# jsourati/nn-active-learning

Hardware: AMD Instinct MI355X
Metric: patches/sec Fisher-scored (32^3, 2-class) (higher is better)
Workload: dtype f32 (fp32 operands split into 16-bit pieces on the 16-bit MFMA, fp32 accumulate: fp16 pairs - 22-23 bits kept per operand, three products - in the conv under the head (forward + backward), in dec1's forward launch and in the other backward launches; bf16 triples - all 24 bits, exact, six products -

## Files before the change

include/alq.h:

```cpp
#ifndef ALQ_H
#define ALQ_H

#include <stddef.h>
#include <stdint.h>

#ifdef __cplusplus
extern "C" {
#endif

typedef struct alq_ctx alq_ctx;
typedef struct alq_model alq_model;

enum { ALQ_OK = 0, ALQ_EINVAL = -1, ALQ_EHIP = -2, ALQ_ENOMEM = -3, ALQ_EUNSUPPORTED = -4 };

enum { ALQ_CONV = 0, ALQ_CONVT = 1, ALQ_POOL = 2, ALQ_FC = 3 };

typedef struct {
    int32_t type;
    int32_t cout;
    int32_t k[3];
    int32_t s[3];
    int32_t relu;
    int32_t skip_src;
} alq_layer_t;
// ... 238 lines not shown

int alq_model_debug_copy(alq_model *m, int layer_idx, int what, int N, float *d_out,
                         int64_t *elems_out);

int alq_debug_set_stamp_buffer(void *d_buf);
int alq_debug_set(int key, int value);
enum {
    ALQ_INFO_SUBNORMALS_OK = 0,
    ALQ_INFO_C3D_FWD = 1,
    ALQ_INFO_C3D_BWD = 2,
    ALQ_INFO_C3D_ONE_ACC = 3,
    ALQ_INFO_FLIP_OVERFLOW = 5,
    ALQ_INFO_F16_DERIVED = 6,
    ALQ_INFO_T3D_FWD = 7,
    ALQ_INFO_T3D_BWD = 8,
    ALQ_INFO_E3D_BWD = 9,
    ALQ_INFO_D3D_FWD = 10,
    ALQ_INFO_D3D_BWD = 11,
    ALQ_INFO_F3D_FWD = 12,
    ALQ_INFO_C3D_BWD_FORM = 13,
    ALQ_INFO_HOST_PACK_ELEMS = 14,
    ALQ_INFO_LSUM = 15,
    ALQ_INFO_DCP_FORM = 16,
    ALQ_INFO_E3D_BWD_FORM = 17
};
int alq_model_engine_info(alq_model *m, int what);

int alq_synth_patches(alq_ctx *ctx, uint64_t seed, int64_t first_id, int64_t n,
                      int64_t elems_per_patch, float *d_out);

enum { ALQ_SRC_F32 = 0, ALQ_SRC_F64 = 1, ALQ_SRC_I16 = 2, ALQ_SRC_U8 = 3 };
int alq_vol_pack(alq_ctx *ctx, const void *const *d_src, int m, int src_type, const int32_t *dims, float *d_out);
int alq_mask_pack(alq_ctx *ctx, const uint8_t *d_src, const int32_t *dims, uint8_t *d_out);
int alq_slice_batch_check(const int32_t *h_dims, int nvol, const int32_t *h_desc, int b, const int32_t *crop, int C);
int alq_slice_batch(alq_ctx *ctx, const float *const *h_vols, const uint8_t *const *h_masks, const int32_t *h_dims, int nvol, int m,
                    const int32_t *h_desc, int b, const int32_t *crop, int C, float *d_X, int32_t *d_lab, int64_t *d_counts);
int64_t alq_slice_batch_trip_rows(void);
int alq_slice_batch_launch_samples(void);

#ifdef __cplusplus
}
#endif
#endif
```

nn-active-learning_amd/csrc/alq_internal.h:

```cpp
#pragma once
#include <hip/hip_runtime.h>

#include <cstdint>
#include <cstdio>
#include <memory>
#include <string>
#include <vector>

#include "alq.h"
#include "engine_switches.h"
#include "model_plan.h"

namespace alq {

#define ALQ_HIP(expr)                                                                     \
    do {                                                                                  \
        hipError_t e_ = (expr);                                                           \
        if (e_ != hipSuccess) {                                                           \
            ::alq::set_error("%s:%d: %s -> %s", __FILE__, __LINE__, #expr,               \
                             hipGetErrorString(e_));                                      \
            return ALQ_EHIP;                                                              \
        }                                                                                 \
    } while (0)

// ... 307 lines not shown
                  int relu, int accumulate, int N, int prof_cls, const Igemm2Fuse *fuse);

struct C3dPlan {
    bool ok = false;
    int D = 0;
    int w_exp = 0;
    int oneacc = 1;
    double flops_per_patch = 0;
    std::vector<unsigned short> h_W;
    void *d_W = nullptr;
    std::vector<unsigned short> h_W7;
    void *d_W7 = nullptr;
};
void c3d_bwd7_pack(C3dPlan *plan, const std::vector<float> &Bmat);
int c3d_subnormals_ok(alq_ctx *ctx);
int c3d_fwd_build(const View &in, const View &out, const int k[3], const int lo[3], const int s[3], C3dPlan *plan);
void c3d_fwd_pack(C3dPlan *plan, const std::vector<float> &Bmat );
int c3d_fwd_launch(alq_ctx *ctx, const C3dPlan &plan, const View &in, const float *bias, int N, const unsigned *amaxA, const unsigned *amaxB,
                   const float *fc_W, float *fc_part, float *asum_part, unsigned char *fc_bits, float flip_tau);
int c3d_bwd_build(const View &fwd_in, const View &fwd_out, const int k[3], const int lo[3], const int s[3], C3dPlan *plan);
void c3d_bwd_pack(C3dPlan *plan, const std::vector<float> &Bmat_fwd );
void c3d_presplit_vec(const float *v, long long F, int e, std::vector<unsigned short> *out);
int c3d_bwd_launch(alq_ctx *ctx, const C3dPlan &plan, int N, const unsigned char *bits, const void *vec16, int e_in, const unsigned char *maskA,
                   float *dB, float *sumA, float *sumB, int rows_per_wave = 8);

struct T3dPlan {
    bool ok = false;
    int kind = 0;
    int w_exp = 0;
    double flops_per_patch = 0;
    std::vector<unsigned short> h_W;
    void *d_W = nullptr;
};
int t3d_build(const View &in, const View &out, const int k[3], const int lo[3], const int s[3], T3dPlan *fwd, T3dPlan *bwd);
void t3d_fwd_pack(T3dPlan *plan, const float *W );
void t3d_bwd_pack(T3dPlan *plan, const float *W);
void t3d8_fwd_pack(T3dPlan *plan, const float *W );
void t3d8_bwd_pack(T3dPlan *plan, const float *W );
int t3d8_bwd_launch(alq_ctx *ctx, const T3dPlan &plan, const View &dout, const View &din, int N, float in_bound, const unsigned char *mask_bits, float *dsum);
int t3d_fwd_launch(alq_ctx *ctx, const T3dPlan &plan, const View &in, const View &out, const float *bias, int N, float *osum, unsigned *out_amax);
int t3d_bwd_launch(alq_ctx *ctx, const T3dPlan &plan, const View &dout, const View &din, int N, float in_bound, const unsigned char *mask_bits,
                   float *dsum);

struct E3dPlan {
    bool ok = false;
    int w_exp = 0;
    double flops_per_patch = 0;
// ... 275 lines not shown
```

nn-active-learning_amd/csrc/c3d.hip:

```cpp
#include "f16_pair.h"
#include "sweep_common.h"

#include <algorithm>
#include <cmath>
#include <cstdlib>
#include <cstring>
#include <vector>

namespace alq {

namespace {
#ifndef C3_SCHED_MASK
#define C3_SCHED_MASK 0
#endif
#ifndef C3_PF
#define C3_PF 8
#endif
#ifndef C3_WD
#define C3_WD 4
#endif
static_assert(C3_PF == 8 || C3_PF == 16, "the ring of staging registers must divide the 16 units of a plane");
static_assert(C3_WD >= 1 && C3_WD <= 8, "weight-difference slices are fetched 1..8 rows ahead");
#ifndef C3_ABL
#define C3_ABL 0
#endif
#ifndef C3_PIPE
#define C3_PIPE 2
#endif
#ifndef C3_FILL_MASK
#define C3_FILL_MASK SW_FILL_MASK
#endif
#ifndef C3_PIN_SUMS
#define C3_PIN_SUMS 1
#endif
#ifndef C3_PEEL
#define C3_PEEL 1
#endif
#ifndef C3_EPI2
#define C3_EPI2 1
#endif
#ifndef C3_BPIPE
#define C3_BPIPE 2
#endif
#ifndef C3_B7PIPE
#define C3_B7PIPE 4
#endif
#ifndef C3_B7PINW
#define C3_B7PINW 0
#endif
#ifndef C3_B7ABL
#define C3_B7ABL 0
#endif

constexpr int C3_TEN = 34 * 16;
constexpr int C3_PIECE = 2 * C3_TEN;
constexpr int C3_ROW = 2 * C3_PIECE;
constexpr int C3_PLANE = 34 * C3_ROW;
constexpr int C3_LDS = 2 * C3_PLANE;
static_assert(C3_LDS <= 160 * 1024, "two plane images must fit the CU's LDS");
}

struct C3FwdArgs {
    const float *inA, *inB;
    const void *W;
    const float *bias;
    const unsigned *amaxA, *amaxB;
    const float *fc_W;
    float *fc_part;
// ... 682 lines not shown
            step(IC<1>{}, pi, 3 * zz + 1, n); ++n;
            step(IC<2>{}, pi, 3 * zz + 2, n); ++n;
        }
        step(IC<0>{}, pi, 30, n); ++n;
        step(IC<1>{}, pi, 31, n); ++n;
        light(IC<0>{}, pi, D - 2);
#else
        for (int zz = 0; zz < 11; ++zz) {
            step(IC<0>{}, pi, 3 * zz, n); ++n;
            step(IC<1>{}, pi, 3 * zz + 1, n); ++n;
            if (zz < 10) { step(IC<2>{}, pi, 3 * zz + 2, n); ++n; }
            else light(IC<0>{}, pi, D - 2);
        }
#endif
    }
    if (np > 0) light(IC<1>{}, np - 1, D - 1);
}

namespace {
constexpr int P7_ROW = 34 * 16;
constexpr int P7_PIECE = 34 * P7_ROW;
constexpr int P7_PLANE = 2 * P7_PIECE + 128;
constexpr int P7_LDS = 4 * P7_PLANE;
static_assert((P7_ROW / 16) % 16 == 2 && (P7_PLANE / 16) % 16 == 0 && P7_LDS <= 160 * 1024, "bank-conflict-free pitches (see above)");
}

__global__ __launch_bounds__(256) __attribute__((amdgpu_waves_per_eu(1, 1))) void c3d_bwd7_kernel(const C3BwdArgs a) {
    extern __shared__ __attribute__((aligned(16))) char lds[];
    constexpr int RW = 8, NU = 4;
    const int tid = threadIdx.x;
    const int lane = tid & 63;
    const int wave = __builtin_amdgcn_readfirstlane(tid >> 6);
    const int lj = lane & 15, lq = lane >> 4;
    const int D = a.D;
    const unsigned plane_v = 32u * 32u;
    const unsigned patch_v = (unsigned)D * plane_v;

    for (int i = tid * 16; i < P7_LDS; i += 256 * 16) *reinterpret_cast<i32x4 *>(lds + i) = i32x4{0, 0, 0, 0};

    f16x8 Wa[3][2], Wb[3][2], Ws[2];
    {
        const i32x4 *Wg = reinterpret_cast<const i32x4 *>(a.W);
#pragma unroll
        for (int dz = 0; dz < 3; ++dz)
#pragma unroll
            for (int pc = 0; pc < 2; ++pc) {
                Wa[dz][pc] = __builtin_bit_cast(f16x8, Wg[((0 + dz) * 2 + pc) * 64 + lane]);
                Wb[dz][pc] = __builtin_bit_cast(f16x8, Wg[((3 + dz) * 2 + pc) * 64 + lane]);
            }
        Ws[0] = __builtin_bit_cast(f16x8, Wg[(6 * 2 + 0) * 64 + lane]);
        Ws[1] = __builtin_bit_cast(f16x8, Wg[(6 * 2 + 1) * 64 + lane]);
#if C3_B7PINW
#pragma unroll
        for (int dz = 0; dz < 3; ++dz)
#pragma unroll
            for (int pc = 0; pc < 2; ++pc) {
                i32x4 x = __builtin_bit_cast(i32x4, Wa[dz][pc]), y = __builtin_bit_cast(i32x4, Wb[dz][pc]);
                asm volatile("" : "+a"(x), "+a"(y));
                Wa[dz][pc] = __builtin_bit_cast(f16x8, x); Wb[dz][pc] = __builtin_bit_cast(f16x8, y);
            }
#endif
    }
    const int offA = wave * RW * P7_ROW + (lq < 3 ? (lj + lq) * 16 : P7_ROW + lj * 16);
    const int offB = (wave * RW + 1) * P7_ROW + (lq < 2 ? (lj + 1 + lq) * 16 : P7_ROW + (lj + lq - 2) * 16);
    const int offS = (wave * RW + 2) * P7_ROW + (lj + 2) * 16;
    const int ringS = lq < 2 ? lq + 2 : 0;
    const int st_lane = (wave * RW + 1 + (lane >> 5)) * P7_ROW + ((lane & 31) + 1) * 16;
    const float inv = __builtin_ldexpf(1.f, -(a.e_in + a.e_w));

    const int G = gridDim.x, b0 = blockIdx.x;
    const int np = b0 < a.N ? (a.N - b0 + G - 1) / G : 0;

    f32x4 acc[3][RW][2];
#pragma unroll
// ... 89 lines not shown
        const unsigned vox = E.pv + E.row_v + (unsigned)i * 32u + (unsigned)hx * 16u;
        __builtin_amdgcn_raw_buffer_store_b128(__builtin_bit_cast(i32x4, val), dB_rsrc, (int)E.off_dB, (int)(vox * 32u), 2 );
        if constexpr (!(C3_B7ABL & 8)) ALQ_STORE_HOLD("v"(val));
        const float t = (val.x + val.y) + (val.z + val.w);
        const unsigned tu = __builtin_bit_cast(unsigned, t);
        const auto sw = hx == 0 ? __builtin_amdgcn_permlane16_swap(tu, 0u, false, false) : __builtin_amdgcn_permlane16_swap(0u, tu, false, false);
        const unsigned s0 = sw[0], s1 = sw[1];
        const float t2 = __builtin_bit_cast(float, s0) + __builtin_bit_cast(float, s1);
        if constexpr (hx == 0) {
            t_keep = t2;
        } else {
            const float ts = t_keep + t2;
            const unsigned rowv = E.pv + E.row_v + (unsigned)i * 32u;
            __builtin_amdgcn_raw_buffer_store_b32(__builtin_bit_cast(int, ts), sA_rsrc, (int)(lq < 2 ? E.off_sum : SW_OOB), (int)(rowv * 4u), 0);
            __builtin_amdgcn_raw_buffer_store_b32(__builtin_bit_cast(int, ts), sB_rsrc, (int)(lq >= 2 ? E.off_sum : SW_OOB), (int)(rowv * 4u), 0);
        }
    };
    auto epi_row = [&](auto S, auto I, const Epi &E) __attribute__((always_inline)) {
        epi_half(S, I, IC<0>{}, E);
        epi_half(S, I, IC<1>{}, E);
    };
    auto s_weights = [&](int kill, f16x8 &sh, f16x8 &sl) __attribute__((always_inline)) {
        const int km = lq == kill ? 0 : -1;
        i32x4 h = __builtin_bit_cast(i32x4, Ws[0]), l = __builtin_bit_cast(i32x4, Ws[1]);
        h.x &= km; h.y &= km; h.z &= km; h.w &= km;
        l.x &= km; l.y &= km; l.z &= km; l.w &= km;
        sh = __builtin_bit_cast(f16x8, h); sl = __builtin_bit_cast(f16x8, l);
    };
    auto mac3 = [&](f32x4 c, const f16x8 &wh, const f16x8 &wl, const f16x8 &bh, const f16x8 &bl) __attribute__((always_inline)) {
        c = __builtin_amdgcn_mfma_f32_16x16x32_f16(wl, bh, c, 0, 0, 0);
        c = __builtin_amdgcn_mfma_f32_16x16x32_f16(wh, bl, c, 0, 0, 0);
        c = __builtin_amdgcn_mfma_f32_16x16x32_f16(wh, bh, c, 0, 0, 0);
        return c;
    };

    auto step = [&](auto RR, int pi, int z, long long n) __attribute__((always_inline)) {
        constexpr int R = decltype(RR)::value;
        constexpr int S_lo = (R + 2) % 3, S_mid = R, S_hi = (R + 1) % 3;
        asm volatile("s_waitcnt lgkmcnt(0)\n\ts_barrier" ::: "memory");
        const int cur = (int)(n & 3) * P7_PLANE;
        const int baseA = offA + cur, baseB = offB + cur;
        const int baseS = offS + (int)((unsigned)((int)(n & 3) + ringS) & 3u) * P7_PLANE;
        const int wbase = st_lane + (int)((n + 1) & 3) * P7_PLANE;
        const Src C1 = src_of(c1_pi), C2 = src_of(c2_pi);
        const unsigned z1 = (unsigned)c1_z, z2 = (unsigned)c2_z;
        const bool ev = z >= 2 || (z == 0 && pi > 0);
        const Epi E = epi_setup(ev, z >= 2 ? pi : pi - 1, z >= 2 ? z - 2 : D - 1);
        f16x8 sh, sl;
        s_weights(z == 1 ? 0 : -1, sh, sl);

        struct Frag { f16x8 ah, al, bh, bl, sh, sl; };
        auto frag = [&](int i, int hx, Frag &f) __attribute__((always_inline)) {
            const int o = i * P7_ROW + hx * 256;
            f.ah = __builtin_bit_cast(f16x8, *reinterpret_cast<const i32x4 *>(lds + baseA + o));
            f.al = __builtin_bit_cast(f16x8, *reinterpret_cast<const i32x4 *>(lds + baseA + o + P7_PIECE));
            f.bh = __builtin_bit_cast(f16x8, *reinterpret_cast<const i32x4 *>(lds + baseB + o));
            f.bl = __builtin_bit_cast(f16x8, *reinterpret_cast<const i32x4 *>(lds + baseB + o + P7_PIECE));
            f.sh = __builtin_bit_cast(f16x8, *reinterpret_cast<const i32x4 *>(lds + baseS + o));
            f.sl = __builtin_bit_cast(f16x8, *reinterpret_cast<const i32x4 *>(lds + baseS + o + P7_PIECE));
        };
        Frag fc, fn;
        frag(0, 0, fc);
        auto row = [&](auto I) __attribute__((always_inline)) {
            constexpr int i = decltype(I)::value;
            __builtin_amdgcn_sched_barrier(0);
            if constexpr (!(C3_B7ABL & 1)) epi_row(IC<S_hi>{}, I, E);
            else { const f32x4 k0 = acc[S_hi][i][0], k1 = acc[S_hi][i][1]; asm volatile("" :: "v"(k0), "v"(k1)); }
            if constexpr ((i & 1) == 0 && !(C3_B7ABL & 2)) {
                stage_unit(wbase, IC<i / 2>{});
                if constexpr (i / 2 + 2 < NU) load_unit(C1, z1, IC<i / 2 + 2>{}); else load_unit(C2, z2, IC<i / 2 + 2 - NU>{});
            }
#pragma unroll
            for (int hx = 0; hx < 2; ++hx) {
                if (hx == 0) frag(i, 1, fn);
                else if (i < RW - 1) frag(i + 1, 0, fn);
                f32x4 c0 = f32x4{0.f, 0.f, 0.f, 0.f}, c1 = acc[S_mid][i][hx], c2 = acc[S_lo][i][hx];
                c0 = mac3(c0, Wa[0][0], Wa[0][1], fc.ah, fc.al);
                c1 = mac3(c1, Wa[1][0], Wa[1][1], fc.ah, fc.al);
                c2 = mac3(c2, Wa[2][0], Wa[2][1], fc.ah, fc.al);
                c0 = mac3(c0, Wb[0][0], Wb[0][1], fc.bh, fc.bl);
                c1 = mac3(c1, Wb[1][0], Wb[1][1], fc.bh, fc.bl);
                c2 = mac3(c2, Wb[2][0], Wb[2][1], fc.bh, fc.bl);
                if constexpr (!(C3_B7ABL & 4)) c2 = mac3(c2, sh, sl, fc.sh, fc.sl);
                acc[S_hi][i][hx] = c0; acc[S_mid][i][hx] = c1; acc[S_lo][i][hx] = c2;
                fc = fn;
            }
#if C3_B7PIPE
#pragma unroll
            for (int m = 0; m < 42; ++m) {
                __builtin_amdgcn_sched_group_barrier(0x008, 1, 0);
                __builtin_amdgcn_sched_group_barrier(C3_FILL_MASK, C3_B7PIPE, 0);
            }
#endif
        };
        row(IC<0>{}); row(IC<1>{}); row(IC<2>{}); row(IC<3>{}); row(IC<4>{}); row(IC<5>{}); row(IC<6>{}); row(IC<7>{});
        {
            const Epi En = epi_setup(z + 1 < D ? z >= 1 : true, pi, z + 1 < D ? z - 1 : D - 2);
            mask_load(En, IC<0>{});
            mask_load(En, IC<1>{});
        }
        c1_pi = c2_pi; c1_z = c2_z;
        advance(c2_pi, c2_z);
    };
    auto light = [&](auto S, auto LAST, int pe, int zo, long long n) __attribute__((always_inline)) {
        constexpr int s = decltype(S)::value;
        constexpr bool last = decltype(LAST)::value != 0;
        const Epi E = epi_setup(true, pe, zo);
        auto rows = [&](auto I) __attribute__((always_inline)) { epi_row(S, I, E); };
        rows(IC<0>{}); rows(IC<1>{}); rows(IC<2>{}); rows(IC<3>{}); rows(IC<4>{}); rows(IC<5>{}); rows(IC<6>{}); rows(IC<7>{});
#pragma unroll
        for (int i = 0; i < RW; ++i) { acc[s][i][0] = f32x4{0.f, 0.f, 0.f, 0.f}; acc[s][i][1] = f32x4{0.f, 0.f, 0.f, 0.f}; }
        if constexpr (last) {
            constexpr int sp = (s + 1) % 3;
            f16x8 sh, sl;
            s_weights(2, sh, sl);
            const int baseS = offS + (int)((unsigned)((int)(n & 3) + ringS) & 3u) * P7_PLANE;
#pragma unroll
            for (int i = 0; i < RW; ++i)
#pragma unroll
                for (int hx = 0; hx < 2; ++hx) {
                    const int o = i * P7_ROW + hx * 256;
                    const f16x8 bh = __builtin_bit_cast(f16x8, *reinterpret_cast<const i32x4 *>(lds + baseS + o));
                    const f16x8 bl = __builtin_bit_cast(f16x8, *reinterpret_cast<const i32x4 *>(lds + baseS + o + P7_PIECE));
                    acc[sp][i][hx] = mac3(acc[sp][i][hx], sh, sl, bh, bl);
                }
        }
        {
            const Epi En = epi_setup(zo == D - 2, pe, D - 1);
            mask_load(En, IC<0>{});
            mask_load(En, IC<1>{});
        }
    };

    __syncthreads();
    if (np > 0) {
        const Src C0 = src_of(0);
        const int wb = st_lane;
        load_unit(C0, 0u, IC<0>{}); load_unit(C0, 0u, IC<1>{});
        stage_unit(wb, IC<0>{}); stage_unit(wb, IC<1>{});
        load_unit(C0, 0u, IC<2>{}); load_unit(C0, 0u, IC<3>{});
        stage_unit(wb, IC<2>{}); stage_unit(wb, IC<3>{});
        c1_pi = 0; c1_z = 0;
        advance(c1_pi, c1_z);
        c2_pi = c1_pi; c2_z = c1_z;
        advance(c2_pi, c2_z);
        const Src C1 = src_of(c1_pi);
        load_unit(C1, (unsigned)c1_z, IC<0>{}); load_unit(C1, (unsigned)c1_z, IC<1>{});
    }
    long long n = 0;
    for (int pi = 0; pi < np; ++pi) {
        for (int zz = 0; zz < 10; ++zz) {
            step(IC<0>{}, pi, 3 * zz, n); ++n;
            step(IC<1>{}, pi, 3 * zz + 1, n); ++n;
            step(IC<2>{}, pi, 3 * zz + 2, n); ++n;
        }
        step(IC<0>{}, pi, 30, n); ++n;
        step(IC<1>{}, pi, 31, n); ++n;
        light(IC<0>{}, IC<1>{}, pi, D - 2, n);
    }
    if (np > 0) light(IC<1>{}, IC<0>{}, np - 1, D - 1, n);
}

__global__ void c3d_subnormal_probe(float *out) {
    f16x8 a, b;
// ... 97 lines not shown
    plan->h_W7.assign((size_t)7 * 2 * 64 * 8, 0);
    for (int f = 0; f < 7; ++f)
        for (int lane = 0; lane < 64; ++lane) {
            const int ci = lane & 15, q = lane >> 4;
            int dz = -1, dy = 0, dx = 0;
            if (f < 3) { dz = f; if (q < 3) { dy = 0; dx = q; } else { dy = 1; dx = 0; } }
            else if (f < 6) { dz = f - 3; const int p = 4 + q; dy = p / 3; dx = p % 3; }
            else if (q < 3) { dz = q; dy = 2; dx = 2; }
            for (int c = 0; c < 8; ++c) {
                float w = 0.f;
                if (dz >= 0) w = Bmat[((size_t)(((2 - dz) * 3 + (2 - dy)) * 3 + (2 - dx)) * 16 + ci) * 8 + c];
                f16_pair_split(w, plan->w_exp, 0, &plan->h_W7[((size_t)(f * 2 + 0) * 64 + lane) * 8 + c], &plan->h_W7[((size_t)(f * 2 + 1) * 64 + lane) * 8 + c]);
            }
        }
}

void c3d_presplit_vec(const float *v, long long F, int e, std::vector<unsigned short> *out) {
    out->assign((size_t)F * 2, 0);
    for (long long vox = 0; vox < F / 8; ++vox)
        for (int c = 0; c < 8; ++c) f16_pair_split(v[vox * 8 + c], e, 0, &(*out)[(size_t)vox * 16 + c], &(*out)[(size_t)vox * 16 + 8 + c]);
}

int c3d_bwd_launch(alq_ctx *ctx, const C3dPlan &plan, int N, const unsigned char *bits, const void *vec16, int e_in, const unsigned char *maskA,
                   float *dB, float *sumA, float *sumB, int rows_per_wave) {
    ALQ_REQUIRE(plan.ok && plan.d_W && plan.D == 32, ALQ_EINVAL, "c3d: backward weights not set");
    ALQ_REQUIRE(bits && vec16 && dB && sumA && sumB, ALQ_EINVAL, "c3d: missing argument");
    SWEEP_REQUIRE_PATCHES(N, "c3d");
    if (N <= 0) return ALQ_OK;
    C3BwdArgs a;
    a.bits = bits; a.vec = vec16; a.W = plan.d_W; a.maskA = maskA; a.dB = dB; a.sumA = sumA; a.sumB = sumB;
    a.N = N; a.D = plan.D; a.e_in = e_in; a.e_w = plan.w_exp;
    ProfScope ps(ctx, PROF_IGEMM_F16, plan.flops_per_patch * N);
    const int rows8 = rows_per_wave == 4 ? 0 : 1;
    if (rows_per_wave == 7 && plan.d_W7) {
        a.W = plan.d_W7;
        return sweep_launch(ctx, c3d_bwd7_kernel, (unsigned)std::min(N, 256), 256, P7_LDS, a);
    }
    if (rows8) return sweep_launch(ctx, c3d_bwd_kernel<true, 8>, (unsigned)std::min(N, 256), 256, 2 * (32 + 2) * B3_ROW + 2 * B3_ROW, a);
    return sweep_launch(ctx, c3d_bwd_kernel<true, 4>, (unsigned)std::min(2 * N, 256), 256, 2 * (16 + 2) * B3_ROW + 2 * B3_ROW, a);
}

}
```

nn-active-learning_amd/csrc/engine_switches.h:

```cpp
#ifndef ALQ_ENGINE_SWITCHES_H
#define ALQ_ENGINE_SWITCHES_H
#include <cstddef>
#include <cstdlib>

namespace alq {

enum Knob {
    KNOB_REPEAT = 0,
    KNOB_FLAGS = 1,
    KNOB_NO_BWD_FUSE = 2,
    KNOB_NO_FWD_FUSE = 3,
    KNOB_NO_V3 = 4,
    KNOB_NO_V4 = 5,
    KNOB_NO_POOL_FIRST = 6,
    KNOB_NO_CONV_POOL = 7,
    KNOB_DCP_NARROW = 8,
    KNOB_E3D_GRID_CAP = 9,
    ALQ_NKNOBS = 10
};

struct EngineSwitches {
    int knobs[ALQ_NKNOBS] = {0, 0, 0, 0, 0, 0, 0, 0, 0, 0};
    int disable_v2 = 0;
    int disable_v3 = 0;
    int disable_v4 = 0;
    int no_fcgemm = 0;
    int no_split = 0;
    int no_wide2d_rule = 0;
    int no_v3_f16 = 0;
    int no_v3_f16_fwd = 0;
    int no_co_split = 0;
    int no_co_split_f16 = 0;
    int no_class_tiles = 0;
    int no_fc_bits = 0;
    int no_fc_fuse = 0;
    int no_fc_f16 = 0;
    int no_fc_f16_fwd = 0;
    int f16_derived_mask = 0;
    int has_f16_derived_mask = 0;
    int no_f16x2 = 0;
    int no_xcd_order = 0;
    int no_fixed = 0;
    int no_bound16 = 0;
    int no_flipfix = 0;
    int no_presplit = 0;
    int no_signs = 0;
    int no_signs0 = 0;
    int f16_fwd_mask = -1;
    int no_f16_derived = 0;
    int no_light_kernels = 0;
    int no_c3d = 0;
    int c3_bwd_rows = 7;
    int no_e3d = 0;
    int e3d_rows = 0;
    int no_d3d = 0;
    int no_d3b = 0;
    int no_f3d = 0;
    int no_t3d = 0;
};

enum SwitchRule {
    SW_PRESENT,
    SW_FIRST_IS_1,
    SW_ATOI_EQ,
    SW_INT,
    SW_ROWS
};

struct SwitchRow {
    const char *env;
    size_t member;
    SwitchRule rule;
    int arg;
};

// ... 47 lines not shown
    ALQ_SW("ALQ_NO_F3D", no_f3d, SW_PRESENT, 0),
    ALQ_SW("ALQ_NO_T3D", no_t3d, SW_PRESENT, 0),
};
#undef ALQ_SW
inline const int kNumSwitchRows = (int)(sizeof(kSwitchTable) / sizeof(kSwitchTable[0]));

inline int &switch_member(EngineSwitches &sw, const SwitchRow &row) {
    return *reinterpret_cast<int *>(reinterpret_cast<char *>(&sw) + row.member);
}

inline EngineSwitches read_engine_switches() {
    EngineSwitches sw;
    for (const SwitchRow &row : kSwitchTable) {
        const char *v = std::getenv(row.env);
        int &dst = switch_member(sw, row);
        switch (row.rule) {
            case SW_PRESENT:    if (v) dst = 1; break;
            case SW_FIRST_IS_1: if (v && v[0] == '1') dst = 1; break;
            case SW_ATOI_EQ:    if (v && std::atoi(v) == row.arg) dst = 1; break;
            case SW_INT:        if (v) dst = std::atoi(v); break;
            case SW_ROWS:       dst = (v && std::atoi(v) == 4) ? 4 : ((v && std::atoi(v) == 8) ? 8 : 7); break;
        }
    }
    return sw;
}

}
#endif
```

nn-active-learning_amd/csrc/igemm2.hip:

```cpp
#include "alq_internal.h"

#include <algorithm>
#include <cmath>
#include <cstring>

namespace alq {

typedef float f32x4 __attribute__((ext_vector_type(4)));
typedef float f32x2 __attribute__((ext_vector_type(2)));

#ifdef ALQ_STAMPS
#define STAMP(var) asm volatile("s_memtime %0\n\ts_waitcnt lgkmcnt(0)" : "=s"(var)::"memory")
#define PHASE_END(idx)                         \
    do {                                       \
        unsigned long long t_now_;             \
        STAMP(t_now_);                         \
        ph[idx] += t_now_ - t_last;            \
        t_last = t_now_;                       \
    } while (0)
#else
#define PHASE_END(idx) do {} while (0)
#endif

constexpr int I2_CBP = 12;
// ... 461 lines not shown
}

void igemm2_pack_weights(Igemm2Plan *p2, const std::vector<float> &Bmat) {
    const Igemm2Args &a = p2->a;
    const int NTW = p2->NTW, Ci = a.Ci, Co = a.Co;
    p2->h_W.assign((size_t)a.nchunks * a.ntaps * NTW * 128, 0.f);
    for (int ch = 0; ch < a.nchunks; ++ch)
        for (int tp = 0; tp < a.ntaps; ++tp)
            for (int nt = 0; nt < NTW; ++nt)
                for (int lane = 0; lane < 64; ++lane)
                    for (int s = 0; s < 2; ++s) {
                        const int c = ch * 8 + 2 * (lane >> 4) + s;
                        const int co = nt * 16 + (lane & 15);
                        if (co < Co)
                            p2->h_W[((((size_t)ch * a.ntaps + tp) * NTW + nt) * 64 + lane) * 2 + s] =
                                Bmat[((size_t)tp * Ci + c) * Co + co];
                    }
}

unsigned long long *g_igemm2_dbg = nullptr;
int g_no_f16x2 = 0;
int g_no_xcd_order = 0;
int g_no_fixed = 0;
int g_dbg_knobs[ALQ_NKNOBS] = {0, 0, 0, 0, 0, 0, 0, 0, 0, 0};

template <int NTW, bool WRES, int GEO, bool SUMS>
static int launch2_s(alq_ctx *ctx, const Igemm2Plan &plan, const Igemm2Args &a, unsigned grid) {
    auto kfn = igemm2_kernel<NTW, WRES, GEO, SUMS>;
    if (plan.lds_bytes > 64 * 1024)
        ALQ_HIP(hipFuncSetAttribute(reinterpret_cast<const void *>(kfn), hipFuncAttributeMaxDynamicSharedMemorySize,
                                    (int)plan.lds_bytes));
    hipLaunchKernelGGL(kfn, dim3(grid), dim3(256), plan.lds_bytes, ctx->stream, a);
    ALQ_HIP(hipGetLastError());
    return ALQ_OK;
}

template <int NTW, bool WRES, int GEO>
static int launch2_t(alq_ctx *ctx, const Igemm2Plan &plan, const Igemm2Args &a, unsigned grid) {
    return (a.osumA || a.osumB) ? launch2_s<NTW, WRES, GEO, true>(ctx, plan, a, grid)
                                : launch2_s<NTW, WRES, GEO, false>(ctx, plan, a, grid);
}

int igemm2_launch(alq_ctx *ctx, const Igemm2Plan &plan, const View &in, const View &out, const float *bias, int relu,
                  int accumulate, int N, int prof_cls, const Igemm2Fuse *fuse) {
    Igemm2Args a = plan.a;
    ALQ_REQUIRE(in.C == a.Ci && in.D == a.ID && in.H == a.IH && in.W == a.IW, ALQ_EINVAL,
                "igemm2: input view does not match plan");
// ... 53 lines not shown
```

nn-active-learning_amd/csrc/model.hip:

```cpp
#include <algorithm>
#include <cmath>
#include <cstring>
#include <string>

#include "model_types.h"

using namespace alq;

static int g_knob_override[ALQ_NKNOBS] = {-1, -1, -1, -1, -1, -1, -1, -1, -1, -1};

static void apply_knobs(const alq_model *m) {
    for (int k = 0; k < ALQ_NKNOBS; ++k) g_dbg_knobs[k] = g_knob_override[k] >= 0 ? g_knob_override[k] : m->sw.knobs[k];
    g_no_f16x2 = m->sw.no_f16x2;
    g_no_xcd_order = m->sw.no_xcd_order;
    g_no_fixed = m->sw.no_fixed;
}

static int gemm_build(const EngineSwitches &sw, const ConvDesc &d, int max_batch, Gemm *g, const G4Geom *g4 = nullptr) {
    ALQ_TRY(igemm_build_plan(d, max_batch, &g->p1));
    if (g4 && !sw.disable_v4) {
        G4Geom gg = *g4;
        gg.flops_per_patch = g->p1.flops_per_patch;
        ALQ_TRY(igemm4_build_plan(gg, max_batch, &g->p4));
    }
    ALQ_TRY(igemm2_build_plan(g->p1, &g->p2));
    ALQ_TRY(direct_build_plan(g->p1, &g->pd));
    if (sw.disable_v2) { g->p2.ok = false; g->pd.ok = false; }
    ALQ_TRY(igemm3_build_plan(g->p2, &g->p3));
    if (d.ID == 1 && d.IH == 1 && d.IW == 1 && d.tz.size() == 1 && d.sm == 1 && d.so == 1 && !sw.no_fcgemm)
        ALQ_TRY(fcgemm_build_plan(d.Ci, d.Co, &g->pfc));
    if (sw.disable_v3) g->p3.ok = false;
    return ALQ_OK;
// ... 884 lines not shown
                    if (next_pool && (sliced || splitv) && (Cs & 3) == 0) {
                        fz.mask = sl.out.p; fz.mask_cs = sl.out.cs; fz.mask_c0 = sl.out.c0; fz.mask_from = 0;
                        fz.mask_bits = (sl.signs_ready && (!prev->spec.relu || prev->signs_ready)) ? sl.out.sg : nullptr;
                        if (splitv) { fz.mask_split = Cs; fz.mask_delta = ly.in.delta; }
                        if (!prev->spec.relu) fz.mask_to = Cs;
                        fz.osumA = sl.dsum; fz.store_from = Cs;
                        sl.dsum_partial = true;
                    }
                }
                fuse = &fz;
            }
            if (ly.dout_bits) {
                fz.in_bits = ly.dout_bits; fz.in_vec = ly.dout_vec; fz.in_vec_amax = ly.dout_vec_amax;
                fz.in_vec16 = m->sw.no_presplit ? nullptr : ly.dout_vec16;
                const unsigned short *vec16c = ly.dout_vec16c;
                ly.dout_bits = nullptr; ly.dout_vec = nullptr; ly.dout_vec16 = nullptr; ly.dout_vec16c = nullptr;
                const bool honoured = fuse != nullptr;
                const bool c3 = c3d_bwd_applies(m, ly, vec16c, fuse, acc);
                m->last.bwd.c3_bwd = c3;
                if (c3) {
                    int ex = 0;
                    (void)std::frexp(fz.in_vec_amax, &ex);
                    ALQ_TRY(c3d_bwd_launch(ctx, ly.c3b, N, reinterpret_cast<const unsigned char *>(fz.in_bits), vec16c, 14 - ex, fz.mask_bits,
                                           ly.din.p + ly.din.delta, fz.osumA, fz.osumB, m->sw.c3_bwd_rows));
                } else {
                    ALQ_TRY(igemm4_launch(ctx, ly.bwd.p4, ly.dout, ly.din, nullptr, 0, acc, N, PROF_IGEMM3_BWD, &fz));
                }
                fused = honoured;
            } else {
                const bool p4_here = fuse && two_slot_allowed() && ly.bwd.p4.ok && !ly.bwd.p4.multi && ly.bwd.p4.a.PT == 1 && !g_no_f16x2;
                bool hand = false;
                if (p4_here && prev_param && !acc && !(prev->dout_bound > 0.f && !m->sw.no_bound16) && prev->pidx > 0 && prev->bwd.p4.ok && !prev->bwd.p4.multi && prev->bwd.p4.a.PT == 1 &&
                    prev->bwd.p4.d_W16 && !prev->dout.split &&
                    ((prev->bwd.p4.NTW == 1 && prev->bwd.p4.fic) || prev->bwd.p4.NTW == 2)) {
                    const size_t len = (size_t)ly.bwd.p4.a.tpg * 4;
                    if (!m->amax_a) { ALQ_TRY(m->dalloc(&m->amax_a, (size_t)m->max_batch)); ALQ_TRY(m->dalloc(&m->amax_b, (size_t)m->max_batch)); }
                    ALQ_TRY(ensure_amax_tiles(m, len));
                    fz.out_amax = m->amax_tiles;
                    fz.amax_from = fz.split > 0 && fz.split < (1 << 29) ? fz.split : 0;
                    hand = true;
                }
                if (p4_here && !acc && ly.dout_amax) fz.in_amax = ly.dout_amax;
                if (p4_here && !acc && !fz.in_amax && ly.dout_bound > 0.f && !m->sw.no_bound16) fz.in_bound = ly.dout_bound;
                if (!fuse && !acc && two_slot_allowed() && ly.bwd.p4.ok && !ly.bwd.p4.multi && ly.bwd.p4.a.PT == 1 && !g_no_f16x2 && !ly.dout_amax &&
                    ly.dout_bound > 0.f && !m->sw.no_bound16 && !g_dbg_knobs[KNOB_NO_BWD_FUSE]) {
                    fz = Igemm2Fuse();
                    fz.in_bound = ly.dout_bound;
// ... 313 lines not shown
            for (const Layer &ly : m->layers)
                if (ly.c3f.ok) return ly.c3f.oneacc;
            return 0;
        case ALQ_INFO_FLIP_OVERFLOW: {
            ALQ_HIP(hipSetDevice(m->ctx->device));
            if (!m->flip_overflow) return 0;
            unsigned h = 0;
            ALQ_HIP(hipMemcpyAsync(&h, m->flip_overflow, sizeof(unsigned), hipMemcpyDeviceToHost, m->ctx->stream));
            ALQ_HIP(hipStreamSynchronize(m->ctx->stream));
            return h > 0x7fffffffu ? 0x7fffffff : (int)h;
        }
        case ALQ_INFO_F16_DERIVED: return m->last.fwd.f16_derived ? 1 : 0;
        case ALQ_INFO_T3D_FWD: return m->last.fwd.t3f;
        case ALQ_INFO_T3D_BWD: return m->last.bwd.t3b;
        case ALQ_INFO_E3D_BWD: return m->last.bwd.e3b;
        case ALQ_INFO_D3D_FWD: return m->last.fwd.d3f;
        case ALQ_INFO_D3D_BWD: return m->last.bwd.d3b;
        case ALQ_INFO_F3D_FWD: return m->last.fwd.f3f;
        case ALQ_INFO_C3D_BWD_FORM: return m->last.bwd.c3_bwd ? m->sw.c3_bwd_rows : 0;
        case ALQ_INFO_HOST_PACK_ELEMS: return m->host_pack_elems > 0x7fffffffll ? 0x7fffffff : (int)m->host_pack_elems;
        case ALQ_INFO_LSUM: return m->last.lsum;
        case ALQ_INFO_DCP_FORM: return m->last.fwd.dcp;
        case ALQ_INFO_E3D_BWD_FORM: return m->last.bwd.e3b_form;
        default: break;
    }
    set_error("alq_model_engine_info: bad argument");
    return ALQ_EINVAL;
}

int alq_debug_set(int key, int value) {
    ALQ_REQUIRE(key >= 0 && key < ALQ_NKNOBS, ALQ_EINVAL, "alq_debug_set: bad key");
    g_knob_override[key] = value > 0 ? value : -1;
    g_dbg_knobs[key] = value;
    return ALQ_OK;
}

int alq_debug_set_stamp_buffer(void *d_buf) {
    g_igemm2_dbg = reinterpret_cast<unsigned long long *>(d_buf);
    return ALQ_OK;
}

}
```

nn-active-learning_amd/csrc/model_types.h:

```cpp
#pragma once
#include <algorithm>

#include "alq_internal.h"

namespace alq {

struct Layer {
    alq_layer_t spec;
    int pidx = -1;
    View in, out;
    View din, dout;
    int lo[3] = {0, 0, 0};
    bool dense_fc_small = false;
    bool dense_head = false;
    int64_t F = 0;
    int64_t w_elems = 0, b_elems = 0;
    float *d_bias = nullptr;
    float *d_Wp = nullptr;
    std::vector<Gemm> fwd;
    std::vector<Gemm> fwd_co;
    int fwd_co_w = 0;
    Igemm4Plan fwd_all;
    Gemm bwd;
    bool has_bwd = false;
// ... 38 lines not shown
    bool out_is_skip_src = false;
    std::vector<std::vector<int>> class_taps;
    std::vector<float> hv_hW;
    int hv_src = 0;
    bool hv_stale = false;
    float *hv_W = nullptr;
    double *hv_A = nullptr, *hv_D = nullptr, *hv_Ra = nullptr, *hv_Rd = nullptr;
};

}

struct PassInfo {
    struct Fwd {
        bool head_fused = false;
        bool c3 = false;
        int t3f = 0;
        int d3f = 0;
        int f3f = 0;
        int dcp = 0;
        bool f16_derived = false;
    } fwd;
    struct Bwd {
        bool c3_bwd = false;
        int t3b = 0;
        int e3b = 0;
        int e3b_form = 0;
        int d3b = 0;
    } bwd;
    int lsum = 0;
    bool call_fisher = false;
};

struct alq_model {
    alq_ctx *ctx = nullptr;
    int max_batch = 0;
    alq::EngineSwitches sw;
    PassInfo last;
    unsigned *amax_a = nullptr, *amax_b = nullptr, *amax_tiles = nullptr;
    unsigned *flip_cnt = nullptr, *flip_list = nullptr;
    int flip_cap = 0;
    unsigned *bound_all = nullptr;
    unsigned *in_amax = nullptr;
    bool v3_fwd_f16 = false;
    unsigned *flip_overflow = nullptr;
    size_t amax_tiles_len = 0;
    int in_dims[4] = {1, 1, 1, 1};
// ... 92 lines not shown
```

Measured before the change: 283,900.

## Run c3d backward kernel with two waves per SIMD and four-row strips

Templates the 7-form c3d backward kernel on rows-per-wave and waves-per-block and makes the default 8 waves (512 threads) with 4 rows each, i.e. two waves per SIMD. To fit the lower register budget, the second fragment set is dropped in favour of a single-set, half-row software pipeline, and the skip-connection weights are moved from registers to an extra LDS slab. The aim is to hide LDS and MFMA latency with a second wave. The cost is more LDS traffic and possibly less instruction-level scheduling per wave. A grid-cap knob and info queries are also added.

```diff
diff --git a/include/alq.h b/include/alq.h
--- a/include/alq.h
+++ b/include/alq.h
@@ -284,7 +284,9 @@
     ALQ_INFO_HOST_PACK_ELEMS = 14,
     ALQ_INFO_LSUM = 15,
     ALQ_INFO_DCP_FORM = 16,
-    ALQ_INFO_E3D_BWD_FORM = 17
+    ALQ_INFO_E3D_BWD_FORM = 17,
+    ALQ_INFO_C3D_BWD_WAVES = 19,
+    ALQ_INFO_C3D_BWD_GRID = 20
 };
 int alq_model_engine_info(alq_model *m, int what);
 
diff --git a/nn-active-learning_amd/csrc/alq_internal.h b/nn-active-learning_amd/csrc/alq_internal.h
--- a/nn-active-learning_amd/csrc/alq_internal.h
+++ b/nn-active-learning_amd/csrc/alq_internal.h
@@ -353,7 +353,8 @@
 void c3d_bwd_pack(C3dPlan *plan, const std::vector<float> &Bmat_fwd );
 void c3d_presplit_vec(const float *v, long long F, int e, std::vector<unsigned short> *out);
 int c3d_bwd_launch(alq_ctx *ctx, const C3dPlan &plan, int N, const unsigned char *bits, const void *vec16, int e_in, const unsigned char *maskA,
-                   float *dB, float *sumA, float *sumB, int rows_per_wave = 8);
+                   float *dB, float *sumA, float *sumB, int rows_per_wave = 8, int waves_per_simd = 1 ,
+                   int *grid_out = nullptr );
 
 struct T3dPlan {
     bool ok = false;
diff --git a/nn-active-learning_amd/csrc/c3d.hip b/nn-active-learning_amd/csrc/c3d.hip
--- a/nn-active-learning_amd/csrc/c3d.hip
+++ b/nn-active-learning_amd/csrc/c3d.hip
@@ -44,6 +44,9 @@
 #endif
 #ifndef C3_B7PIPE
 #define C3_B7PIPE 4
+#endif
+#ifndef C3_B7PIPE2
+#define C3_B7PIPE2 2
 #endif
 #ifndef C3_B7PINW
 #define C3_B7PINW 0
@@ -772,12 +775,18 @@
 constexpr int P7_PIECE = 34 * P7_ROW;
 constexpr int P7_PLANE = 2 * P7_PIECE + 128;
 constexpr int P7_LDS = 4 * P7_PLANE;
-static_assert((P7_ROW / 16) % 16 == 2 && (P7_PLANE / 16) % 16 == 0 && P7_LDS <= 160 * 1024, "bank-conflict-free pitches (see above)");
-}
-
-__global__ __launch_bounds__(256) __attribute__((amdgpu_waves_per_eu(1, 1))) void c3d_bwd7_kernel(const C3BwdArgs a) {
+constexpr int P7_WS = 2 * 64 * 16;
+static_assert((P7_ROW / 16) % 16 == 2 && (P7_PLANE / 16) % 16 == 0 && P7_LDS + P7_WS <= 160 * 1024, "bank-conflict-free pitches (see above)");
+}
+
+template <int RW, int NW>
+__global__ __launch_bounds__(NW * 64) __attribute__((amdgpu_waves_per_eu(NW / 4, NW / 4))) void c3d_bwd7_kernel(const C3BwdArgs a) {
     extern __shared__ __attribute__((aligned(16))) char lds[];
-    constexpr int RW = 8, NU = 4;
+    static_assert(RW * NW == 32 && (NW == 4 || NW == 8), "the waves' strips of RW rows tile the 32 rows of a plane");
+    constexpr int NU = RW / 2;
+    constexpr int FSETS = NW == 4 ? 2 : 1;
+    constexpr int PIPE = NW == 4 ? C3_B7PIPE : C3_B7PIPE2;
+    constexpr bool WS_LDS = NW == 8;
     const int tid = threadIdx.x;
     const int lane = tid & 63;
     const int wave = __builtin_amdgcn_readfirstlane(tid >> 6);
@@ -786,7 +795,7 @@
     const unsigned plane_v = 32u * 32u;
     const unsigned patch_v = (unsigned)D * plane_v;
 
-    for (int i = tid * 16; i < P7_LDS; i += 256 * 16) *reinterpret_cast<i32x4 *>(lds + i) = i32x4{0, 0, 0, 0};
+    for (int i = tid * 16; i < P7_LDS; i += NW * 64 * 16) *reinterpret_cast<i32x4 *>(lds + i) = i32x4{0, 0, 0, 0};
 
     f16x8 Wa[3][2], Wb[3][2], Ws[2];
     {
@@ -800,6 +809,12 @@
             }
         Ws[0] = __builtin_bit_cast(f16x8, Wg[(6 * 2 + 0) * 64 + lane]);
         Ws[1] = __builtin_bit_cast(f16x8, Wg[(6 * 2 + 1) * 64 + lane]);
+        if constexpr (WS_LDS) {
+            if (wave == 0) {
+                *reinterpret_cast<i32x4 *>(lds + P7_LDS + lane * 16) = __builtin_bit_cast(i32x4, Ws[0]);
+                *reinterpret_cast<i32x4 *>(lds + P7_LDS + 1024 + lane * 16) = __builtin_bit_cast(i32x4, Ws[1]);
+            }
+        }
 #if C3_B7PINW
 #pragma unroll
         for (int dz = 0; dz < 3; ++dz)
@@ -935,7 +950,13 @@
     };
     auto s_weights = [&](int kill, f16x8 &sh, f16x8 &sl) __attribute__((always_inline)) {
         const int km = lq == kill ? 0 : -1;
-        i32x4 h = __builtin_bit_cast(i32x4, Ws[0]), l = __builtin_bit_cast(i32x4, Ws[1]);
+        i32x4 h, l;
+        if constexpr (WS_LDS) {
+            h = *reinterpret_cast<const i32x4 *>(lds + P7_LDS + lane * 16);
+            l = *reinterpret_cast<const i32x4 *>(lds + P7_LDS + 1024 + lane * 16);
+        } else {
+            h = __builtin_bit_cast(i32x4, Ws[0]); l = __builtin_bit_cast(i32x4, Ws[1]);
+        }
         h.x &= km; h.y &= km; h.z &= km; h.w &= km;
         l.x &= km; l.y &= km; l.z &= km; l.w &= km;
         sh = __builtin_bit_cast(f16x8, h); sl = __builtin_bit_cast(f16x8, l);
@@ -963,20 +984,72 @@
         s_weights(z == 1 ? 0 : -1, sh, sl);
 
         struct Frag { f16x8 ah, al, bh, bl, sh, sl; };
-        auto frag = [&](int i, int hx, Frag &f) __attribute__((always_inline)) {
+        auto frag_s = [&](int i, int hx, Frag &f) __attribute__((always_inline)) {
+            const int o = i * P7_ROW + hx * 256;
+            f.sh = __builtin_bit_cast(f16x8, *reinterpret_cast<const i32x4 *>(lds + baseS + o));
+            f.sl = __builtin_bit_cast(f16x8, *reinterpret_cast<const i32x4 *>(lds + baseS + o + P7_PIECE));
+        };
+        auto frag_a = [&](int i, int hx, Frag &f) __attribute__((always_inline)) {
             const int o = i * P7_ROW + hx * 256;
             f.ah = __builtin_bit_cast(f16x8, *reinterpret_cast<const i32x4 *>(lds + baseA + o));
             f.al = __builtin_bit_cast(f16x8, *reinterpret_cast<const i32x4 *>(lds + baseA + o + P7_PIECE));
+        };
+        auto frag_b = [&](int i, int hx, Frag &f) __attribute__((always_inline)) {
+            const int o = i * P7_ROW + hx * 256;
             f.bh = __builtin_bit_cast(f16x8, *reinterpret_cast<const i32x4 *>(lds + baseB + o));
             f.bl = __builtin_bit_cast(f16x8, *reinterpret_cast<const i32x4 *>(lds + baseB + o + P7_PIECE));
-            f.sh = __builtin_bit_cast(f16x8, *reinterpret_cast<const i32x4 *>(lds + baseS + o));
-            f.sl = __builtin_bit_cast(f16x8, *reinterpret_cast<const i32x4 *>(lds + baseS + o + P7_PIECE));
         };
+        auto frag_ab = [&](int i, int hx, Frag &f) __attribute__((always_inline)) { frag_a(i, hx, f); frag_b(i, hx, f); };
+        auto frag = [&](int i, int hx, Frag &f) __attribute__((always_inline)) { frag_ab(i, hx, f); frag_s(i, hx, f); };
         Frag fc, fn;
-        frag(0, 0, fc);
+        if constexpr (FSETS == 2) frag(0, 0, fc);
+        if constexpr (FSETS == 1) frag_a(0, 0, fc);
+        auto mfma_half = [&](auto I, int hx) __attribute__((always_inline)) {
+            constexpr int i = decltype(I)::value;
+            f32x4 c0 = f32x4{0.f, 0.f, 0.f, 0.f}, c1 = acc[S_mid][i][hx], c2 = acc[S_lo][i][hx];
+            c0 = mac3(c0, Wa[0][0], Wa[0][1], fc.ah, fc.al);
+            c1 = mac3(c1, Wa[1][0], Wa[1][1], fc.ah, fc.al);
+            c2 = mac3(c2, Wa[2][0], Wa[2][1], fc.ah, fc.al);
+            c0 = mac3(c0, Wb[0][0], Wb[0][1], fc.bh, fc.bl);
+            c1 = mac3(c1, Wb[1][0], Wb[1][1], fc.bh, fc.bl);
+            c2 = mac3(c2, Wb[2][0], Wb[2][1], fc.bh, fc.bl);
+            if constexpr (!(C3_B7ABL & 4)) c2 = mac3(c2, sh, sl, fc.sh, fc.sl);
+            acc[S_hi][i][hx] = c0; acc[S_mid][i][hx] = c1; acc[S_lo][i][hx] = c2;
+        };
         auto row = [&](auto I) __attribute__((always_inline)) {
             constexpr int i = decltype(I)::value;
             __builtin_amdgcn_sched_barrier(0);
+            if constexpr (FSETS == 1) {
+                static_assert(NU == 2, "two units per plane and wave");
+#pragma unroll
+                for (int hx = 0; hx < 2; ++hx) {
+                    frag_b(i, hx, fc);
+                    if constexpr (!(C3_B7ABL & 4)) frag_s(i, hx, fc);
+                    if constexpr (!(C3_B7ABL & 1)) {
+                        if (hx == 0) epi_half(IC<S_hi>{}, I, IC<0>{}, E);
+                        else epi_half(IC<S_hi>{}, I, IC<1>{}, E);
+                    } else { const f32x4 k0 = acc[S_hi][i][hx]; asm volatile("" :: "v"(k0)); }
+                    if (hx == 0) frag_a(i, 1, fn);
+                    else if (i < RW - 1) frag_a(i + 1, 0, fn);
+                    if constexpr ((i & 1) == 0 && !(C3_B7ABL & 2)) {
+                        if (hx == 1) {
+                            stage_unit(wbase, IC<i / 2>{});
+                            load_unit(C2, z2, IC<i / 2>{});
+                        }
+                    }
+                    mfma_half(I, hx);
+                    fc.ah = fn.ah; fc.al = fn.al;
+                    if constexpr (PIPE != 0) {
+#pragma unroll
+                        for (int m = 0; m < 21; ++m) {
+                            __builtin_amdgcn_sched_group_barrier(0x008, 1, 0);
+                            __builtin_amdgcn_sched_group_barrier(C3_FILL_MASK, PIPE, 0);
+                        }
+                        __builtin_amdgcn_sched_barrier(0);
+                    }
+                }
+                return;
+            }
             if constexpr (!(C3_B7ABL & 1)) epi_row(IC<S_hi>{}, I, E);
             else { const f32x4 k0 = acc[S_hi][i][0], k1 = acc[S_hi][i][1]; asm volatile("" :: "v"(k0), "v"(k1)); }
             if constexpr ((i & 1) == 0 && !(C3_B7ABL & 2)) {
@@ -987,26 +1060,19 @@
             for (int hx = 0; hx < 2; ++hx) {
                 if (hx == 0) frag(i, 1, fn);
                 else if (i < RW - 1) frag(i + 1, 0, fn);
-                f32x4 c0 = f32x4{0.f, 0.f, 0.f, 0.f}, c1 = acc[S_mid][i][hx], c2 = acc[S_lo][i][hx];
-                c0 = mac3(c0, Wa[0][0], Wa[0][1], fc.ah, fc.al);
-                c1 = mac3(c1, Wa[1][0], Wa[1][1], fc.ah, fc.al);
-                c2 = mac3(c2, Wa[2][0], Wa[2][1], fc.ah, fc.al);
-                c0 = mac3(c0, Wb[0][0], Wb[0][1], fc.bh, fc.bl);
-                c1 = mac3(c1, Wb[1][0], Wb[1][1], fc.bh, fc.bl);
-                c2 = mac3(c2, Wb[2][0], Wb[2][1], fc.bh, fc.bl);
-                if constexpr (!(C3_B7ABL & 4)) c2 = mac3(c2, sh, sl, fc.sh, fc.sl);
-                acc[S_hi][i][hx] = c0; acc[S_mid][i][hx] = c1; acc[S_lo][i][hx] = c2;
+                mfma_half(I, hx);
                 fc = fn;
             }
-#if C3_B7PIPE
-#pragma unroll
-            for (int m = 0; m < 42; ++m) {
-                __builtin_amdgcn_sched_group_barrier(0x008, 1, 0);
-                __builtin_amdgcn_sched_group_barrier(C3_FILL_MASK, C3_B7PIPE, 0);
-            }
-#endif
+            if constexpr (PIPE != 0) {
+#pragma unroll
+                for (int m = 0; m < 42; ++m) {
+                    __builtin_amdgcn_sched_group_barrier(0x008, 1, 0);
+                    __builtin_amdgcn_sched_group_barrier(C3_FILL_MASK, PIPE, 0);
+                }
+            }
         };
-        row(IC<0>{}); row(IC<1>{}); row(IC<2>{}); row(IC<3>{}); row(IC<4>{}); row(IC<5>{}); row(IC<6>{}); row(IC<7>{});
+        row(IC<0>{}); row(IC<1>{}); row(IC<2>{}); row(IC<3>{});
+        if constexpr (RW == 8) { row(IC<4>{}); row(IC<5>{}); row(IC<6>{}); row(IC<7>{}); }
         {
             const Epi En = epi_setup(z + 1 < D ? z >= 1 : true, pi, z + 1 < D ? z - 1 : D - 2);
             mask_load(En, IC<0>{});
@@ -1020,7 +1086,8 @@
         constexpr bool last = decltype(LAST)::value != 0;
         const Epi E = epi_setup(true, pe, zo);
         auto rows = [&](auto I) __attribute__((always_inline)) { epi_row(S, I, E); };
-        rows(IC<0>{}); rows(IC<1>{}); rows(IC<2>{}); rows(IC<3>{}); rows(IC<4>{}); rows(IC<5>{}); rows(IC<6>{}); rows(IC<7>{});
+        rows(IC<0>{}); rows(IC<1>{}); rows(IC<2>{}); rows(IC<3>{});
+        if constexpr (RW == 8) { rows(IC<4>{}); rows(IC<5>{}); rows(IC<6>{}); rows(IC<7>{}); }
 #pragma unroll
         for (int i = 0; i < RW; ++i) { acc[s][i][0] = f32x4{0.f, 0.f, 0.f, 0.f}; acc[s][i][1] = f32x4{0.f, 0.f, 0.f, 0.f}; }
         if constexpr (last) {
@@ -1051,8 +1118,10 @@
         const int wb = st_lane;
         load_unit(C0, 0u, IC<0>{}); load_unit(C0, 0u, IC<1>{});
         stage_unit(wb, IC<0>{}); stage_unit(wb, IC<1>{});
-        load_unit(C0, 0u, IC<2>{}); load_unit(C0, 0u, IC<3>{});
-        stage_unit(wb, IC<2>{}); stage_unit(wb, IC<3>{});
+        if constexpr (NU == 4) {
+            load_unit(C0, 0u, IC<2>{}); load_unit(C0, 0u, IC<3>{});
+            stage_unit(wb, IC<2>{}); stage_unit(wb, IC<3>{});
+        }
         c1_pi = 0; c1_z = 0;
         advance(c1_pi, c1_z);
         c2_pi = c1_pi; c2_z = c1_z;
@@ -1196,10 +1265,11 @@
 }
 
 int c3d_bwd_launch(alq_ctx *ctx, const C3dPlan &plan, int N, const unsigned char *bits, const void *vec16, int e_in, const unsigned char *maskA,
-                   float *dB, float *sumA, float *sumB, int rows_per_wave) {
+                   float *dB, float *sumA, float *sumB, int rows_per_wave, int waves_per_simd, int *grid_out) {
     ALQ_REQUIRE(plan.ok && plan.d_W && plan.D == 32, ALQ_EINVAL, "c3d: backward weights not set");
     ALQ_REQUIRE(bits && vec16 && dB && sumA && sumB, ALQ_EINVAL, "c3d: missing argument");
     SWEEP_REQUIRE_PATCHES(N, "c3d");
+    if (grid_out) *grid_out = 0;
     if (N <= 0) return ALQ_OK;
     C3BwdArgs a;
     a.bits = bits; a.vec = vec16; a.W = plan.d_W; a.maskA = maskA; a.dB = dB; a.sumA = sumA; a.sumB = sumB;
@@ -1208,8 +1278,13 @@
     const int rows8 = rows_per_wave == 4 ? 0 : 1;
     if (rows_per_wave == 7 && plan.d_W7) {
         a.W = plan.d_W7;
-        return sweep_launch(ctx, c3d_bwd7_kernel, (unsigned)std::min(N, 256), 256, P7_LDS, a);
+        unsigned g = (unsigned)std::min(N, 256);
+        if (g_dbg_knobs[KNOB_C3B7_GRID_CAP] > 0) g = std::min<unsigned>(g, (unsigned)g_dbg_knobs[KNOB_C3B7_GRID_CAP]);
+        if (grid_out) *grid_out = (int)g;
+        if (waves_per_simd == 2) return sweep_launch(ctx, c3d_bwd7_kernel<4, 8>, g, 512, P7_LDS + P7_WS, a);
+        return sweep_launch(ctx, c3d_bwd7_kernel<8, 4>, g, 256, P7_LDS, a);
     }
+    if (grid_out) *grid_out = rows8 ? std::min(N, 256) : std::min(2 * N, 256);
     if (rows8) return sweep_launch(ctx, c3d_bwd_kernel<true, 8>, (unsigned)std::min(N, 256), 256, 2 * (32 + 2) * B3_ROW + 2 * B3_ROW, a);
     return sweep_launch(ctx, c3d_bwd_kernel<true, 4>, (unsigned)std::min(2 * N, 256), 256, 2 * (16 + 2) * B3_ROW + 2 * B3_ROW, a);
 }
diff --git a/nn-active-learning_amd/csrc/engine_switches.h b/nn-active-learning_amd/csrc/engine_switches.h
--- a/nn-active-learning_amd/csrc/engine_switches.h
+++ b/nn-active-learning_amd/csrc/engine_switches.h
@@ -16,11 +16,12 @@
     KNOB_NO_CONV_POOL = 7,
     KNOB_DCP_NARROW = 8,
     KNOB_E3D_GRID_CAP = 9,
-    ALQ_NKNOBS = 10
+    KNOB_C3B7_GRID_CAP = 10,
+    ALQ_NKNOBS = 11
 };
 
 struct EngineSwitches {
-    int knobs[ALQ_NKNOBS] = {0, 0, 0, 0, 0, 0, 0, 0, 0, 0};
+    int knobs[ALQ_NKNOBS] = {0, 0, 0, 0, 0, 0, 0, 0, 0, 0, 0};
     int disable_v2 = 0;
     int disable_v3 = 0;
     int disable_v4 = 0;
@@ -51,6 +52,7 @@
     int no_light_kernels = 0;
     int no_c3d = 0;
     int c3_bwd_rows = 7;
+    int c3_bwd_waves = 2;
     int no_e3d = 0;
     int e3d_rows = 0;
     int no_d3d = 0;
@@ -144,6 +146,7 @@
             case SW_ROWS:       dst = (v && std::atoi(v) == 4) ? 4 : ((v && std::atoi(v) == 8) ? 8 : 7); break;
         }
     }
+    if (const char *v = std::getenv("ALQ_C3D_BWD_WAVES")) sw.c3_bwd_waves = std::atoi(v) == 1 ? 1 : 2;
     return sw;
 }
 
diff --git a/nn-active-learning_amd/csrc/igemm2.hip b/nn-active-learning_amd/csrc/igemm2.hip
--- a/nn-active-learning_amd/csrc/igemm2.hip
+++ b/nn-active-learning_amd/csrc/igemm2.hip
@@ -507,7 +507,7 @@
 int g_no_f16x2 = 0;
 int g_no_xcd_order = 0;
 int g_no_fixed = 0;
-int g_dbg_knobs[ALQ_NKNOBS] = {0, 0, 0, 0, 0, 0, 0, 0, 0, 0};
+int g_dbg_knobs[ALQ_NKNOBS] = {0, 0, 0, 0, 0, 0, 0, 0, 0, 0, 0};
 
 template <int NTW, bool WRES, int GEO, bool SUMS>
 static int launch2_s(alq_ctx *ctx, const Igemm2Plan &plan, const Igemm2Args &a, unsigned grid) {
diff --git a/nn-active-learning_amd/csrc/model.hip b/nn-active-learning_amd/csrc/model.hip
--- a/nn-active-learning_amd/csrc/model.hip
+++ b/nn-active-learning_amd/csrc/model.hip
@@ -7,7 +7,7 @@
 
 using namespace alq;
 
-static int g_knob_override[ALQ_NKNOBS] = {-1, -1, -1, -1, -1, -1, -1, -1, -1, -1};
+static int g_knob_override[ALQ_NKNOBS] = {-1, -1, -1, -1, -1, -1, -1, -1, -1, -1, -1};
 
 static void apply_knobs(const alq_model *m) {
     for (int k = 0; k < ALQ_NKNOBS; ++k) g_dbg_knobs[k] = g_knob_override[k] >= 0 ? g_knob_override[k] : m->sw.knobs[k];
@@ -938,7 +938,7 @@
                     int ex = 0;
                     (void)std::frexp(fz.in_vec_amax, &ex);
                     ALQ_TRY(c3d_bwd_launch(ctx, ly.c3b, N, reinterpret_cast<const unsigned char *>(fz.in_bits), vec16c, 14 - ex, fz.mask_bits,
-                                           ly.din.p + ly.din.delta, fz.osumA, fz.osumB, m->sw.c3_bwd_rows));
+                                           ly.din.p + ly.din.delta, fz.osumA, fz.osumB, m->sw.c3_bwd_rows, m->sw.c3_bwd_waves, &m->last.bwd.c3b_grid));
                 } else {
                     ALQ_TRY(igemm4_launch(ctx, ly.bwd.p4, ly.dout, ly.din, nullptr, 0, acc, N, PROF_IGEMM3_BWD, &fz));
                 }
@@ -1298,6 +1298,8 @@
         case ALQ_INFO_LSUM: return m->last.lsum;
         case ALQ_INFO_DCP_FORM: return m->last.fwd.dcp;
         case ALQ_INFO_E3D_BWD_FORM: return m->last.bwd.e3b_form;
+        case ALQ_INFO_C3D_BWD_WAVES: return m->last.bwd.c3_bwd ? (m->sw.c3_bwd_rows == 7 ? m->sw.c3_bwd_waves : 1) : 0;
+        case ALQ_INFO_C3D_BWD_GRID: return m->last.bwd.c3_bwd ? m->last.bwd.c3b_grid : 0;
         default: break;
     }
     set_error("alq_model_engine_info: bad argument");
diff --git a/nn-active-learning_amd/csrc/model_types.h b/nn-active-learning_amd/csrc/model_types.h
--- a/nn-active-learning_amd/csrc/model_types.h
+++ b/nn-active-learning_amd/csrc/model_types.h
@@ -84,6 +84,7 @@
     } fwd;
     struct Bwd {
         bool c3_bwd = false;
+        int c3b_grid = 0;
         int t3b = 0;
         int e3b = 0;
         int e3b_form = 0;
```

Measured after the change: 291,700, median of 6. +2.7%, better.
